# BurntSushi/suffix

Hardware: NVIDIA H100
Metric: MB/s input text indexed (SA+LCP build) (higher is better)
Workload: dtype u32

## Files before the change

suffix_b200/csrc/b200sa.cu:

```cuda
#include <cuda_runtime.h>
#include <stdint.h>
#include <stdio.h>
#include <stdlib.h>
#include <string.h>

#include <string>
#include <vector>

#include "../../include/b200sa.h"
#include "../../include/b200sa_internal.h"
#include "common.cuh"
#include "classify.cuh"
#include "classify2.cuh"
#include "induce.cuh"
#include "induce2.cuh"
#include "induce3.cuh"
#include "induce4.cuh"
#include "induce5.cuh"
#include "induce6.cuh"
#include "pipeline_kernels.cuh"
#include "lms_sort.cuh"
#include "shard.cuh"
#include "tree.cuh"
#include "nccl_dyn.h"
// ... 93 lines not shown

static inline uint32_t cdiv(uint64_t a, uint64_t b) { return (uint32_t)((a + b - 1) / b); }

static int mark(b200sa_ctx *c, const char *name) {
    if (!c->timing) return B200SA_OK;
    if (c->events_used == c->event_pool.size()) {
        cudaEvent_t e;
        CU_TRY(c, cudaEventCreate(&e));
        c->event_pool.push_back(e);
    }
    cudaEvent_t e = c->event_pool[c->events_used++];
    CU_TRY(c, cudaEventRecord(e, c->stream));
    c->marks.push_back({name, e});
    return B200SA_OK;
}
static void begin_call(b200sa_ctx *c, void *stream) {
    c->stream = stream ? (cudaStream_t)stream : c->own_stream;
    c->marks.clear();
    c->events_used = 0;
    c->launches = 0;
    c->last_error.clear();
}
static void l2_window(b200sa_ctx *c, const void *p, size_t bytes);
static int end_call(b200sa_ctx *c) {
    if (c->l2_persist) l2_window(c, nullptr, 0);
    c->stats.kernel_launches = c->launches;
    c->stats.workspace_bytes = c->ws_bytes;
    c->phase_names.clear();
    c->phase_ms.clear();
    if (c->timing && c->marks.size() >= 2) {
        CU_TRY(c, cudaEventSynchronize(c->marks.back().second));
        for (size_t i = 0; i + 1 < c->marks.size(); i++) {
            float ms = 0;
            CU_TRY(c, cudaEventElapsedTime(&ms, c->marks[i].second, c->marks[i + 1].second));
            c->phase_names.push_back(c->marks[i].first);
            c->phase_ms.push_back(ms);
        }
    }
    return B200SA_OK;
}

template <class... KArgs, class... Args>
static inline void launch_k(b200sa_ctx *c, void (*kern)(KArgs...), uint32_t grid, Args... args) {
    kern<<<grid, BLK, 0, c->stream>>>(args...);
    c->launches++;
}
#define LAUNCH(ctx, kern, grid, ...) launch_k((ctx), kern, (grid), __VA_ARGS__)

static int read_words(b200sa_ctx *c, const uint32_t *dsrc, int count) {
    CU_TRY(c, cudaMemcpyAsync(c->h_pin, dsrc, sizeof(uint32_t) * count, cudaMemcpyDeviceToHost, c->stream));
    CU_TRY(c, cudaStreamSynchronize(c->stream));
    return B200SA_OK;
}

static int scan_state_for(b200sa_ctx *c, uint32_t nb, ScanState *S) {
    size_t need = (size_t)nb * 28 + 64;
    if (c->scan_state.cap < need) {
        TRY(ensure(c, c->scan_state, need * 2));
        CU_TRY(c, cudaMemsetAsync(c->scan_state.p, 0, c->scan_state.cap, c->stream));
        c->scan_tiles_cap = (uint32_t)((c->scan_state.cap - 64) / 28);
    }
    uint8_t *basep = ptr<uint8_t>(c->scan_state);
    S->ticket = reinterpret_cast<uint32_t *>(basep);
    S->agg = reinterpret_cast<unsigned long long *>(basep + 64);
    S->incl = S->agg + c->scan_tiles_cap;
    S->pk = S->incl + c->scan_tiles_cap;
    S->flag = reinterpret_cast<uint32_t *>(S->pk + c->scan_tiles_cap);
    c->scan_epoch += 2;
    S->epoch = c->scan_epoch;
    return B200SA_OK;
}

template <class Op, class InF, class OutF>
static int dev_scan(b200sa_ctx *c, InF in, OutF out, uint64_t n, typename Op::T *d_total) {
    typedef typename Op::T T;
    if (n == 0) {
        if (d_total) CU_TRY(c, cudaMemsetAsync(d_total, 0, sizeof(T), c->stream));
        return B200SA_OK;
    }
    uint32_t nb = cdiv(n, SCAN_CHUNK);
    ScanState S;
    TRY(scan_state_for(c, nb, &S));
    LAUNCH(c, (k_scan_lb<Op, InF, OutF>), nb, in, out, n, nb, S, d_total);
    CU_TRY(c, cudaGetLastError());
    return B200SA_OK;
}

static inline uint32_t grid_cap(const b200sa_ctx *c) { return (uint32_t)c->sm_count * 8u; }

template <class DigF, class MoveF>
static int radix_pass(b200sa_ctx *c, DigF dig, MoveF mv, uint64_t n) {
    if (n == 0) return B200SA_OK;
    uint32_t tiles = cdiv(n, TILE);
    uint32_t nb = tiles < grid_cap(c) ? tiles : grid_cap(c);
    uint32_t tpb = cdiv(tiles, nb);
    nb = cdiv(tiles, tpb);
    TRY(ensure(c, c->radix_cnt, (size_t)256 * nb * 4));
    uint32_t *cnt = ptr<uint32_t>(c->radix_cnt);
    LAUNCH(c, (k_radix_hist<DigF>), nb, dig, n, tpb, cnt);
    TRY((dev_scan<OpSum>(c, InArray{cnt}, OutStoreExcl{cnt}, (uint64_t)256 * nb, nullptr)));
    LAUNCH(c, (k_radix_scatter<DigF, MoveF>), nb, dig, mv, n, tpb, cnt);
    CU_TRY(c, cudaGetLastError());
    return B200SA_OK;
}

template <class K, int OSI>
static int sort_pairs_t(b200sa_ctx *c, K *ka, uint32_t *va, K *kb, uint32_t *vb, uint64_t n, int bits,
                      K **kout, uint32_t **vout) {
    *kout = ka;
    *vout = va;
    if (n == 0 || bits <= 0) return B200SA_OK;
    int npass = (bits + 7) / 8;
    if (npass > OS_MAX_PASSES) npass = OS_MAX_PASSES;
    uint32_t tiles = cdiv(n, OSI * BLK);
    size_t status_bytes = (size_t)tiles * 256 * 8;
    TRY(ensure(c, c->os_hist, OS_MAX_PASSES * 256 * 4 + 64));
    TRY(ensure(c, c->os_status, status_bytes));
    uint32_t *ghist = ptr<uint32_t>(c->os_hist);
    uint32_t *ticket = ghist + OS_MAX_PASSES * 256;
    CU_TRY(c, cudaMemsetAsync(ghist, 0, OS_MAX_PASSES * 256 * 4 + 64, c->stream));
    uint32_t hb = cdiv(n, TILE) < grid_cap(c) ? cdiv(n, TILE) : grid_cap(c);
    {
        size_t shm = (size_t)NWARP * npass * 256 * 4;
        auto kfn = k_os_hist<K, LoadArr<K>>;
        CU_TRY(c, cudaFuncSetAttribute(kfn, cudaFuncAttributeMaxDynamicSharedMemorySize, (int)(NWARP * OS_MAX_PASSES * 256 * 4)));
        kfn<<<hb, BLK, shm, c->stream>>>(LoadArr<K>{ka}, n, npass, 0u, ghist, (K *)nullptr);
        c->launches++;
    }
    LAUNCH(c, k_os_scan, (uint32_t)npass, ghist);
    for (int p = 0; p < npass; p++) {
        CU_TRY(c, cudaMemsetAsync(c->os_status.p, 0, status_bytes, c->stream));
        LAUNCH(c, (k_os_pass<K, LoadArr<K>, LoadArr<uint32_t>, OSI>), tiles, LoadArr<K>{ka}, LoadArr<uint32_t>{va}, kb, vb, n,
               (uint32_t)(8 * p), ghist + p * 256,
               reinterpret_cast<volatile unsigned long long *>(c->os_status.p), ticket + p);
        K *tk = ka; ka = kb; kb = tk;
        uint32_t *tv = va; va = vb; vb = tv;
    }
    CU_TRY(c, cudaGetLastError());
    *kout = ka;
    *vout = va;
    return B200SA_OK;
}

template <class K>
static int sort_pairs(b200sa_ctx *c, K *ka, uint32_t *va, K *kb, uint32_t *vb, uint64_t n, int bits,
                      K **kout, uint32_t **vout) {
    if (n >= (1u << 20) && !getenv("B200SA_SORT_NARROW"))
        return sort_pairs_t<K, (sizeof(K) == 4 ? 16 : 12)>(c, ka, va, kb, vb, n, bits, kout, vout);
    return sort_pairs_t<K, ITEMS>(c, ka, va, kb, vb, n, bits, kout, vout);
}

template <class K, class KeyF, class ValF, int OSI = ITEMS>
static int sort_pairs_from(b200sa_ctx *c, KeyF keyf, ValF valf, K *ka, uint32_t *va, K *kb, uint32_t *vb, uint64_t n,
                           int bits, K **kout, uint32_t **vout) {
    *kout = ka;
    *vout = va;
    if (n == 0) return B200SA_OK;
    int npass = (bits + 7) / 8;
    if (npass < 1) npass = 1;
    if (npass > OS_MAX_PASSES) npass = OS_MAX_PASSES;
    uint32_t tiles = cdiv(n, OSI * BLK);
    size_t status_bytes = (size_t)tiles * 256 * 8;
    TRY(ensure(c, c->os_hist, OS_MAX_PASSES * 256 * 4 + 64));
    TRY(ensure(c, c->os_status, status_bytes));
    uint32_t *ghist = ptr<uint32_t>(c->os_hist);
    uint32_t *ticket = ghist + OS_MAX_PASSES * 256;
    CU_TRY(c, cudaMemsetAsync(ghist, 0, OS_MAX_PASSES * 256 * 4 + 64, c->stream));
    uint32_t hb = cdiv(n, TILE) < grid_cap(c) ? cdiv(n, TILE) : grid_cap(c);
    {
        size_t shm = (size_t)NWARP * npass * 256 * 4;
        auto kfn = k_os_hist<K, KeyF>;
        CU_TRY(c, cudaFuncSetAttribute(kfn, cudaFuncAttributeMaxDynamicSharedMemorySize, (int)(NWARP * OS_MAX_PASSES * 256 * 4)));
        kfn<<<hb, BLK, shm, c->stream>>>(keyf, n, npass, 0u, ghist, kb);
        c->launches++;
    }
    LAUNCH(c, k_os_scan, (uint32_t)npass, ghist);
    volatile unsigned long long *status = reinterpret_cast<volatile unsigned long long *>(c->os_status.p);
    CU_TRY(c, cudaMemsetAsync(c->os_status.p, 0, status_bytes, c->stream));
    LAUNCH(c, (k_os_pass<K, LoadArr<K>, ValF, OSI>), tiles, LoadArr<K>{kb}, valf, ka, va, n, 0u, ghist, status, ticket);
    for (int p = 1; p < npass; p++) {
        CU_TRY(c, cudaMemsetAsync(c->os_status.p, 0, status_bytes, c->stream));
        LAUNCH(c, (k_os_pass<K, LoadArr<K>, LoadArr<uint32_t>, OSI>), tiles, LoadArr<K>{ka}, LoadArr<uint32_t>{va}, kb, vb, n,
               (uint32_t)(8 * p), ghist + p * 256, status, ticket + p);
        K *tk = ka; ka = kb; kb = tk;
        uint32_t *tv = va; va = vb; vb = tv;
    }
    CU_TRY(c, cudaGetLastError());
    *kout = ka;
    *vout = va;
    return B200SA_OK;
}

static int bit_length(uint64_t x) {
    int b = 0;
    while (x) { b++; x >>= 1; }
    return b;
}

static int doubling_rounds(b200sa_ctx *c, uint32_t m, uint32_t na, uint32_t *asuf, uint32_t *ascratch, uint64_t h,
                           uint32_t *rounds_io, const uint32_t *names_arr = nullptr, uint32_t kgram = 0,
                           uint32_t bw = 0) {
    uint32_t *sa_r = ptr<uint32_t>(c->sa_r), *rank = ptr<uint32_t>(c->rank);
    uint32_t *apos = ptr<uint32_t>(c->p0), *apos_next = ptr<uint32_t>(c->p1);
    uint32_t *G0 = ptr<uint32_t>(c->g0), *G1 = ptr<uint32_t>(c->g1), *agrp = G0;
    uint32_t *d_na = ptr<uint32_t>(c->small);
    uint32_t rounds = *rounds_io;
    if (na > 0) {
        TRY(ensure(c, c->k64a, (size_t)na * 8));
        TRY(ensure(c, c->k64b, (size_t)na * 8));
    }
    int b2 = bit_length(m);
    bool try_local = getenv("B200SA_NO_LOCAL_SORT") == nullptr;
    static const char *kSortNames[] = {"rsa_sort1", "rsa_sort2", "rsa_sort3", "rsa_sort4", "rsa_sort5", "rsa_sortN"};
    static const char *kScanNames[] = {"rsa_scan1", "rsa_scan2", "rsa_scan3", "rsa_scan4", "rsa_scan5", "rsa_scanN"};
    while (na > 0) {
        rounds++;
        { uint32_t ri = rounds - *rounds_io; TRY(mark(c, kSortNames[ri <= 5 ? ri - 1 : 5])); }
        if (rounds > 40) { c->last_error = "doubling did not converge"; return B200SA_ERR_INTERNAL; }
        uint64_t *KA = ptr<uint64_t>(c->k64a), *KB = ptr<uint64_t>(c->k64b), *K2;
        uint32_t hh = h > 0xffffffffull ? 0xffffffffu : (uint32_t)h;
        bool first = (names_arr != nullptr) && rounds == *rounds_io + 1 && kgram >= 2;
        int bits = 2 * b2;
        if (first) {
            LAUNCH(c, (k_multi_key_list<uint64_t>), cdiv(na, BLK), names_arr, m, asuf, na, kgram, bw, KA);
            bits = (int)(kgram * bw);
        } else {
            LAUNCH(c, k_pair_keys, cdiv(na, BLK), agrp, asuf, rank, na, m, hh, (uint32_t)b2, KA);
        }
        uint32_t *Vsorted = nullptr;
        bool sorted_locally = false;
        bool use_local = !first && try_local;
        if (use_local) {
            CU_TRY(c, cudaMemsetAsync(d_na + 24, 0, 16, c->stream));
            uint32_t stride = na / 4096u; if (stride < 1) stride = 1;
            uint32_t samples = cdiv(na, stride);
            LAUNCH(c, k_group_probe, cdiv(samples, BLK), KA, na, (uint32_t)b2, stride, d_na + 25);
            TRY(read_words(c, d_na + 25, 2));
            if (c->h_pin[0] * 20u > samples) use_local = false;
        }
        if (use_local) {
            LAUNCH(c, k_group_local_sort, cdiv(na, BLK), KA, asuf, na, (uint32_t)b2, KB, ascratch, d_na + 24);
            TRY(read_words(c, d_na + 24, 1));
            if (c->h_pin[0] == 0) { K2 = KB; Vsorted = ascratch; sorted_locally = true; }
            else try_local = false;
        }
        if (!sorted_locally) TRY(sort_pairs<uint64_t>(c, KA, asuf, KB, ascratch, na, bits, &K2, &Vsorted));
        uint32_t *Vother = (Vsorted == asuf) ? ascratch : asuf;
        { uint32_t ri = rounds - *rounds_io; TRY(mark(c, kScanNames[ri <= 5 ? ri - 1 : 5])); }
        TRY((dev_scan<OpMaxSum>(c, InGroupActive<uint64_t>{K2, apos, na},
                                OutGroupRankCompact{Vsorted, apos, rank, sa_r, apos_next, Vother, G0}, na,
                                reinterpret_cast<unsigned long long *>(d_na + 16))));
        TRY(read_words(c, d_na + 16, 1));
        na = c->h_pin[0];
        if (getenv("B200SA_TRACE")) fprintf(stderr, "[b200sa] doubling round %u: h=%llu -> active %u of %u\n", rounds, (unsigned long long)h, na, m);
        asuf = Vother; ascratch = Vsorted;
        uint32_t *t = apos; apos = apos_next; apos_next = t;
        agrp = G0;
        if (first) h = kgram; else h *= 2;
    }
    *rounds_io = rounds;
    return B200SA_OK;
}


static int reduced_sa(b200sa_ctx *c, uint32_t *R, uint32_t m, uint32_t names, uint32_t *rounds_out) {
    TRY(ensure(c, c->sa_r, (size_t)m * 4));
    TRY(ensure(c, c->k32b, (size_t)m * 4));
    TRY(ensure(c, c->v0, (size_t)m * 4));
    TRY(ensure(c, c->v1, (size_t)m * 4));
    TRY(ensure(c, c->p0, (size_t)m * 4));
    TRY(ensure(c, c->p1, (size_t)m * 4));
    TRY(ensure(c, c->g0, (size_t)m * 4));
    TRY(ensure(c, c->g1, (size_t)m * 4));
    TRY(ensure(c, c->rank, (size_t)m * 4));
    TRY(ensure(c, c->small, 256));
    uint32_t *sa_r = ptr<uint32_t>(c->sa_r), *rank = ptr<uint32_t>(c->rank);
    uint32_t *V0 = ptr<uint32_t>(c->v0), *V1 = ptr<uint32_t>(c->v1);
    uint32_t *P0 = ptr<uint32_t>(c->p0), *P1 = ptr<uint32_t>(c->p1);
    uint32_t *G0 = ptr<uint32_t>(c->g0), *G1 = ptr<uint32_t>(c->g1);
    uint32_t *d_na = ptr<uint32_t>(c->small);
    uint32_t rounds = 0;

    LAUNCH(c, k_iota, cdiv(m, BLK), V0, m);
    int bm = bit_length(m);
    int bw = bit_length(names);
    if (bw < 1) bw = 1;
    uint32_t k0 = 1;
    if (bw + 3 < bm) {
        k0 = (uint32_t)((bm + 2 + bw - 1) / bw);
        if ((int)k0 * bw > 64) k0 = 64 / bw;
    }
    if (const char *e = getenv("B200SA_K0")) { int v = atoi(e); if (v >= 1 && v * bw <= 64) k0 = (uint32_t)v; }
    uint32_t *Vs;
    uint32_t na = 0;
    if ((int)k0 * bw <= 32) {
        uint32_t *KA = ptr<uint32_t>(c->k32b), *Ks;
        LAUNCH(c, (k_multi_key<uint32_t>), cdiv(m, BLK), R, m, k0, (uint32_t)bw, KA);
        TRY(sort_pairs<uint32_t>(c, KA, V0, R, V1, m, (int)k0 * bw, &Ks, &Vs));
        TRY((dev_scan<OpMax>(c, InGroupStart<uint32_t>{Ks, nullptr}, OutGroupRank{Vs, nullptr, G1, rank, sa_r}, m, nullptr)));
        uint32_t *Vf = (Vs == V0) ? V1 : V0;
        TRY((dev_scan<OpSum>(c, InActive<uint32_t>{Ks, m}, OutCompactActive{nullptr, Vs, G1, P0, Vf, G0}, m, d_na)));
    } else {
        TRY(ensure(c, c->k64a, (size_t)m * 8));
        TRY(ensure(c, c->k64b, (size_t)m * 8));
        uint64_t *KA = ptr<uint64_t>(c->k64a), *KB = ptr<uint64_t>(c->k64b), *Ks;
        LAUNCH(c, (k_multi_key<uint64_t>), cdiv(m, BLK), R, m, k0, (uint32_t)bw, KA);
        TRY(sort_pairs<uint64_t>(c, KA, V0, KB, V1, m, (int)k0 * bw, &Ks, &Vs));
        TRY((dev_scan<OpMax>(c, InGroupStart<uint64_t>{Ks, nullptr}, OutGroupRank{Vs, nullptr, G1, rank, sa_r}, m, nullptr)));
        uint32_t *Vf = (Vs == V0) ? V1 : V0;
        TRY((dev_scan<OpSum>(c, InActive<uint64_t>{Ks, m}, OutCompactActive{nullptr, Vs, G1, P0, Vf, G0}, m, d_na)));
    }
    uint32_t *Vfree = (Vs == V0) ? V1 : V0;
    TRY(read_words(c, d_na, 1));
    na = c->h_pin[0];
    TRY(doubling_rounds(c, m, na, Vfree, Vs, k0, &rounds));
    if (rounds_out) *rounds_out = rounds;
    return B200SA_OK;
}

static void l2_window(b200sa_ctx *c, const void *p, size_t bytes) {
    if (!c->l2_persist || c->l2_max_window == 0) return;
    cudaStreamAttrValue v;
    memset(&v, 0, sizeof v);
    v.accessPolicyWindow.base_ptr = const_cast<void *>(p);
    v.accessPolicyWindow.num_bytes = bytes < c->l2_max_window ? bytes : c->l2_max_window;
    v.accessPolicyWindow.hitRatio = bytes ? 1.0f : 0.0f;
    v.accessPolicyWindow.hitProp = cudaAccessPropertyPersisting;
    v.accessPolicyWindow.missProp = cudaAccessPropertyStreaming;
    if (cudaStreamSetAttribute(c->stream, cudaStreamAttributeAccessPolicyWindow, &v) != cudaSuccess) cudaGetLastError();
}

static int pack_text(b200sa_ctx *c, const uint8_t *text, uint64_t n, uint32_t sigma) {
    uint32_t *tab = ptr<uint32_t>(c->tables);
    c->bits = 8;
    c->ptext = text;
    c->sigma = sigma;
    if (getenv("B200SA_NOPACK")) return B200SA_OK;
    if (sigma <= 4) c->bits = 2; else if (sigma <= 16) c->bits = 4; else return B200SA_OK;
    uint32_t cpw = 32 / c->bits;
    uint64_t words = (n + cpw - 1) / cpw;
    TRY(ensure(c, c->packed, words * 4 + 32));
    if (c->bits == 2) LAUNCH(c, (k_pack<2>), cdiv(words, BLK), text, n, tab + T_CODE, ptr<uint32_t>(c->packed));
    else LAUNCH(c, (k_pack<4>), cdiv(words, BLK), text, n, tab + T_CODE, ptr<uint32_t>(c->packed));
    CU_TRY(c, cudaGetLastError());
    c->ptext = c->packed.p;
    if (words * 4 <= c->l2_set_aside) l2_window(c, c->packed.p, words * 4 + 8);
    return B200SA_OK;
}

static uint32_t window_chars(uint32_t sigma, int bits, uint64_t *range_out) {
    if (bits == 2) { *range_out = 1ull << 32; return 16; }
    if (sigma < 2) sigma = 2;
    uint32_t cap = bits == 4 ? 13u : 8u, k = 0;
    uint64_t r = 1;
    while (k < cap && r * sigma <= (1ull << 32)) { r *= sigma; k++; }
    *range_out = r;
    return k;
}

template <int BITS>
static int lms_direct_sort_t(b200sa_ctx *c, uint32_t n, uint32_t m, uint32_t **list_out, bool *done) {
    *done = false;
    uint64_t range = 0;
    LmsWin W;
    W.ptext = c->ptext; W.code_of = ptr<uint32_t>(c->tables) + T_CODE; W.n = n;
    W.sigma = BITS == 2 ? 4u : c->sigma;
    W.kc = window_chars(c->sigma, BITS, &range);
    const uint32_t kc = W.kc;
    TRY(ensure(c, c->k32b, (size_t)m * 4));
    TRY(ensure(c, c->reduced, (size_t)m * 4));
    TRY(ensure(c, c->v0, (size_t)m * 4));
    TRY(ensure(c, c->v1, (size_t)m * 4));
    TRY(ensure(c, c->small, 4096));
    uint32_t *sm = ptr<uint32_t>(c->small);
    uint32_t *Ks, *Ps;
    TRY(mark(c, "lms_sort"));
    {
        const char *e = getenv("B200SA_SORT_ITEMS");
        const bool wide = e ? atoi(e) == 16 : (m >= (1u << 20) && !getenv("B200SA_SORT_NARROW"));
        LmsKeyDesc<BITS> kf{W, ptr<uint32_t>(c->lmsdesc)};
        LmsValDesc vf{ptr<uint32_t>(c->lmsdesc)};
        if (wide)
            TRY((sort_pairs_from<uint32_t, LmsKeyDesc<BITS>, LmsValDesc, 16>(c, kf, vf, ptr<uint32_t>(c->k32b), ptr<uint32_t>(c->v0),
                                                                             ptr<uint32_t>(c->reduced), ptr<uint32_t>(c->v1), m,
                                                                             bit_length(range - 1), &Ks, &Ps)));
        else
            TRY((sort_pairs_from<uint32_t, LmsKeyDesc<BITS>, LmsValDesc, ITEMS>(c, kf, vf, ptr<uint32_t>(c->k32b), ptr<uint32_t>(c->v0),
                                                                                ptr<uint32_t>(c->reduced), ptr<uint32_t>(c->v1), m,
                                                                                bit_length(range - 1), &Ks, &Ps)));
    }
    TRY(mark(c, "lms_groups"));
    TRY(ensure(c, c->p0, (size_t)m * 4));
    TRY(ensure(c, c->p1, (size_t)m * 4));
    TRY(ensure(c, c->g0, (size_t)m * 4));
    TRY(ensure(c, c->g1, (size_t)m * 4));
    TRY(ensure(c, c->sa_r, (size_t)m * 4));
    TRY(ensure(c, c->rank, (size_t)m * 4));
    uint32_t *slotA = ptr<uint32_t>(c->p0), *slotB = ptr<uint32_t>(c->p1);
    uint32_t *grpA = ptr<uint32_t>(c->g0), *grpB = ptr<uint32_t>(c->g1);
    uint32_t *posA = ptr<uint32_t>(c->sa_r), *posB = ptr<uint32_t>(c->rank);
    unsigned long long *d_tot = reinterpret_cast<unsigned long long *>(sm + 16);
    {
        size_t fw = ((size_t)m + 31) / 32 + 1;
        TRY(ensure(c, c->flag, fw * 4));
        uint32_t *forced = ptr<uint32_t>(c->flag);
        CU_TRY(c, cudaMemsetAsync(forced, 0, fw * 4, c->stream));
        CU_TRY(c, cudaMemsetAsync(sm + 16, 0, 8, c->stream));
        LAUNCH(c, (k_lms_mark_trunc<BITS>), 1u, W, ptr<uint32_t>(c->lmsdesc), m, Ks, Ps, kc, forced);
        if (getenv("B200SA_GROUPS_GENERIC")) {
            InLmsActive1 in1{Ks, forced, m};
            TRY((dev_scan<OpSum>(c, in1, OutLmsCompact1{in1, Ps, slotA, posA, grpA}, m, sm + 16)));
        } else {
            uint32_t nt = cdiv(m, LG_TILE);
            ScanState S;
            TRY(scan_state_for(c, nt, &S));
            LAUNCH(c, k_lms_groups1, nt, Ks, Ps, forced, m, nt, S, slotA, posA, grpA, sm + 16);
            CU_TRY(c, cudaGetLastError());
        }
    }
    TRY(read_words(c, sm + 16, 1));
    uint32_t na = c->h_pin[0];
    c->stats.names = m - na;
    uint32_t rounds = 1;
    uint32_t max_rounds = BITS == 8 ? 16u : 8u;
    if (const char *e = getenv("B200SA_DIRECT_ROUNDS")) { int v = atoi(e); if (v >= 1) max_rounds = (uint32_t)v; }
    if (getenv("B200SA_TRACE")) fprintf(stderr, "[b200sa] direct LMS sort: kc=%u, round 1 leaves %u of %u tied\n", kc, na, m);
    const bool force = getenv("B200SA_DIRECT_FORCE") != nullptr;
    if (!force && (uint64_t)na * 1000 > (uint64_t)m * 999 && m > 64) return B200SA_OK;
    if (na > 0)
        TRY((dev_scan<OpMax>(c, InArray{grpA}, OutMaxInPlace{grpA}, na, nullptr)));
    uint64_t h = kc;
    const bool allow_local = getenv("B200SA_NO_LOCAL_SORT") == nullptr;
    const int gbits = 32 + bit_length(m);
    while (na > 0) {
        if (rounds >= max_rounds) return B200SA_OK;
        rounds++;
        {
            static const char *kNames[] = {"lms_refine2", "lms_refine3", "lms_refine4", "lms_refine5", "lms_refineN"};
            TRY(mark(c, kNames[rounds - 2 < 4 ? rounds - 2 : 4]));
        }
        TRY(ensure(c, c->k64a, (size_t)na * 8));
        TRY(ensure(c, c->k64b, (size_t)na * 8));
        TRY(ensure(c, c->sorted, (size_t)m * 4));
        uint64_t *KA = ptr<uint64_t>(c->k64a), *KB = ptr<uint64_t>(c->k64b), *K2 = nullptr;
        uint32_t *scratch = ptr<uint32_t>(c->sorted), *P2 = nullptr;
        LAUNCH(c, (k_lms_refine_keys<BITS>), cdiv(na, BLK), W, posA, grpA, na, (uint32_t)h, KA);
        const uint32_t span = (uint32_t)(h + kc > 0xffffffffull ? 0xffffffffull : h + kc);
        bool local_ok = false;
        bool try_local = allow_local;
        if (try_local && na >= (1u << 20)) {
            CU_TRY(c, cudaMemsetAsync(sm + 24, 0, 16, c->stream));
            uint32_t stride = na / 4096u; if (stride < 1) stride = 1;
            uint32_t samples = cdiv(na, stride);
            LAUNCH(c, k_group_probe, cdiv(samples, BLK), KA, na, 32u, stride, sm + 25);
            TRY(read_words(c, sm + 25, 2));
            if (c->h_pin[0] * 20u > samples) try_local = false;
        }
        if (try_local) {
            CU_TRY(c, cudaMemsetAsync(sm + 24, 0, 4, c->stream));
            LAUNCH(c, k_group_local_sort, cdiv(na, BLK), KA, posA, na, 32u, KB, scratch, sm + 24);
            TRY((dev_scan<OpMaxSum>(c, InLmsGroupR{KB, scratch, slotA, na, n, span},
                                    OutLmsCompactR{scratch, slotA, Ps, slotB, posB, grpB}, na, d_tot)));
            TRY(read_words(c, sm + 16, 9));
            local_ok = c->h_pin[8] == 0;
        }
        if (!local_ok) {
            TRY(sort_pairs<uint64_t>(c, KA, posA, KB, scratch, na, gbits, &K2, &P2));
            TRY((dev_scan<OpMaxSum>(c, InLmsGroupR{K2, P2, slotA, na, n, span},
                                    OutLmsCompactR{P2, slotA, Ps, slotB, posB, grpB}, na, d_tot)));
            TRY(read_words(c, sm + 16, 1));
        }
        uint32_t na_next = c->h_pin[0];
        if (getenv("B200SA_TRACE")) fprintf(stderr, "[b200sa] direct LMS sort: round %u (h=%llu): %u -> %u tied\n", rounds, (unsigned long long)h, na, na_next);
        if (!force && (uint64_t)na_next * 100 > (uint64_t)na * 85 && (uint64_t)na_next * 64 > m) return B200SA_OK;
        na = na_next;
        uint32_t *t;
        t = slotA; slotA = slotB; slotB = t;
        t = posA; posA = posB; posB = t;
        t = grpA; grpA = grpB; grpB = t;
        h += kc;
    }
    c->stats.doubling_rounds = rounds;
    *list_out = Ps;
    *done = true;
    return B200SA_OK;
}
static int lms_direct_sort(b200sa_ctx *c, uint32_t n, uint32_t m, uint32_t **list_out, bool *done) {
    if (c->bits == 2) return lms_direct_sort_t<2>(c, n, m, list_out, done);
    if (c->bits == 4) return lms_direct_sort_t<4>(c, n, m, list_out, done);
    return lms_direct_sort_t<8>(c, n, m, list_out, done);
}

static int induce_variant_env() {
    const char *e = getenv("B200SA_INDUCE");
    return e ? atoi(e) : 0;
}
static int induce_variant(int bits) {
    int v = induce_variant_env();
    if (v == 2 && bits < 8) return 2;
    if (v == 1) return 1;
    if (bits == 2) return (v >= 3 && v <= 5) ? v : 6;
    return 1;
}
static const void *induce_fn_v(bool spass, int bits, int variant) {
    if (variant == 6 && bits == 2) return spass ? (const void *)k_induce6<true> : (const void *)k_induce6<false>;
    if (variant == 5 && bits == 2) return spass ? (const void *)k_induce5<true> : (const void *)k_induce5<false>;
    if (variant == 4 && bits == 2) return spass ? (const void *)k_induce4<true> : (const void *)k_induce4<false>;
    if (variant == 3 && bits == 2) return spass ? (const void *)k_induce3<true> : (const void *)k_induce3<false>;
    if (variant == 2 && bits == 2) return spass ? (const void *)k_induce2<true, 2> : (const void *)k_induce2<false, 2>;
    if (variant == 2 && bits == 4) return spass ? (const void *)k_induce2<true, 4> : (const void *)k_induce2<false, 4>;
    if (bits == 2) return spass ? (const void *)k_induce<true, 2> : (const void *)k_induce<false, 2>;
    if (bits == 4) return spass ? (const void *)k_induce<true, 4> : (const void *)k_induce<false, 4>;
    return spass ? (const void *)k_induce<true, 8> : (const void *)k_induce<false, 8>;
}
static int launch_induce(b200sa_ctx *c, bool spass, const uint8_t *text, uint32_t n, uint32_t *sa,
                         const uint32_t *lms, uint32_t m) {
    (void)m;
    uint32_t *tab = ptr<uint32_t>(c->tables);
    InduceArgs A;
    A.text = text; A.ptext = c->ptext; A.alpha = tab + T_ALPHA;
    A.n = n; A.sa = sa; A.pred = ptr<uint8_t>(c->pred);
    A.lms = lms; A.lms_pred = ptr<uint8_t>(c->lmspred);
    A.bstart = tab + T_BSTART; A.Lcnt = tab + T_LCNT; A.Scnt = tab + T_SCNT; A.lms_off = tab + T_LMSOFF;
    A.blk_cnt = ptr<uint32_t>(c->blkcnt);
    uint32_t *sm = ptr<uint32_t>(c->small);
    A.g_fill = sm + 64; A.g_state = reinterpret_cast<int32_t *>(sm + 320); A.err = sm + 32;
    A.run_scratch = ptr<uint32_t>(c->runscr);
    A.run_alive = A.run_scratch + TILE;
    A.cmd = sm + 336;
    A.steplog = nullptr;
    A.blocklog_step = 0;
    A.carry = 0;
    { static int rs = -1; if (rs < 0) { const char *e = getenv("B200SA_RUN_STREAK"); rs = e ? atoi(e) : 0; } A.run_streak = (uint32_t)rs; }
    if (getenv("B200SA_STEPLOG")) {
        if (ensure(c, c->steplog, 8192 * 8) == B200SA_OK) {
            A.steplog = ptr<unsigned long long>(c->steplog);
            if (const char *e = getenv("B200SA_BLOCKLOG")) {
                int ps = 0, st = 0;
                if (sscanf(e, "%d:%d", &ps, &st) == 2 && ps == (spass ? 1 : 0)) A.blocklog_step = (uint32_t)st + 1u;
            }
            if (!spass) cudaMemsetAsync(c->steplog.p, 0, 8, c->stream);
        }
    }
    void *args[] = {&A};
    int variant = induce_variant(c->bits);
    if (variant >= 3 && (((uintptr_t)sa | (uintptr_t)lms) & 15) != 0) variant = 1;
    A.carry = (variant >= 5) ? 2 : (variant == 4 ? 1 : 0);
    int bi = c->bits == 2 ? 0 : (c->bits == 4 ? 1 : 2);
    int blocks = c->cur_induce_blocks, cap = c->sm_count * c->induce_occ_v[variant][bi];
    if (blocks > cap) blocks = cap;
    A.cascade = 0;
    if (variant == 6 && !getenv("B200SA_NO_CASCADE")) {
        A.cascade = (uint32_t)blocks * (uint32_t)TILE;
        if (const char *e = getenv("B200SA_CASCADE_MAX")) { long v = atol(e); if (v >= 0 && (uint64_t)v < A.cascade) A.cascade = (uint32_t)v; }
    }
    CU_TRY(c, cudaLaunchCooperativeKernel(induce_fn_v(spass, c->bits, variant), dim3(blocks), dim3(BLK), args, 0, c->stream));
    c->launches++;
    return B200SA_OK;
}

static int post_classify(b200sa_ctx *c, const uint8_t *text, uint64_t n, uint32_t sigma) {
    TRY(pack_text(c, text, n, sigma));
    int bps = sigma <= 16 ? 3 : (sigma <= 64 ? 2 : 1);
    if (c->induce_bps_env) bps = c->induce_bps_env;
    int occ_here = c->induce_occ[c->bits == 2 ? 0 : (c->bits == 4 ? 1 : 2)];
    if (bps > occ_here) bps = occ_here;
    if (bps < 1) bps = 1;
    c->cur_induce_blocks = c->sm_count * bps;
    return B200SA_OK;
}

static int classify_fused_dev(b200sa_ctx *c, const uint8_t *text, uint64_t n, uint32_t *m_out,
                              ShardEdge edge = ShardEdge{-1, -1, ST_L}, bool pack = true) {
    uint64_t nw = (n + 31) / 32;
    uint32_t nbc = cdiv(nw, CLS_WORDS);
    TRY(ensure(c, c->stype, nw * 4));
    TRY(ensure(c, c->lmsb, nw * 4));
    TRY(ensure(c, c->tables, T_END * 4));
    TRY(ensure(c, c->small, 4096));
    TRY(ensure(c, c->lmsdesc, (size_t)(n / 2 + 2) * 4));
    if (c->cls_state.cap < (size_t)nbc * 4) {
        TRY(ensure(c, c->cls_state, (size_t)nbc * 8));
// ... 1300 lines not shown
```

suffix_b200/csrc/lms_sort.cuh:

```cuda
#pragma once
#include "classify.cuh"

namespace b200sa {

struct LmsWin {
    const void *ptext;
    const uint32_t *code_of;
    uint32_t n, sigma, kc;
};

__device__ __forceinline__ uint32_t rev_pairs(uint32_t x) {
    uint32_t y = __brev(x);
    return ((y & 0x55555555u) << 1) | ((y >> 1) & 0x55555555u);
}

template <int BITS>
__device__ __forceinline__ uint32_t lms_window(const LmsWin &W, uint32_t p) {
    const uint32_t left = W.n - p;
    if (BITS == 2) {
        if (left == 0) return 0u;
        uint32_t x = text_bits<2>(W.ptext, p);
        if (left < 16u) x &= (1u << (2u * left)) - 1u;
        return rev_pairs(x);
    } else if (BITS == 4) {
        if (left == 0) return 0u;
        uint32_t lo = text_bits<4>(W.ptext, p);
        uint32_t hi = (W.kc > 8u && left > 8u) ? text_bits<4>(W.ptext, p + 8u) : 0u;
        uint32_t key = 0;
        for (uint32_t i = 0; i < W.kc; i++) {
            uint32_t c = (i < 8u ? (lo >> (4u * i)) : (hi >> (4u * (i - 8u)))) & 15u;
            key = key * W.sigma + (i < left ? c : 0u);
        }
        return key;
    } else {
        const uint8_t *t = reinterpret_cast<const uint8_t *>(W.ptext);
        uint32_t key = 0;
        if (W.sigma == 256u) {
#pragma unroll
            for (uint32_t i = 0; i < 4u; i++) key = (key << 8) | (i < left ? (uint32_t)__ldg(t + p + i) : 0u);
            return key;
        }
        for (uint32_t i = 0; i < W.kc; i++) {
            uint32_t c = i < left ? __ldg(W.code_of + __ldg(t + p + i)) : 0u;
            key = key * W.sigma + c;
        }
        return key;
    }
}

template <int BITS>
struct LmsKeyDesc {
    LmsWin W; const uint32_t *lmsdesc;
    __device__ __forceinline__ uint32_t operator()(uint64_t i) const { return lms_window<BITS>(W, __ldg(lmsdesc + i)); }
    __device__ __forceinline__ uint32_t at(uint64_t, uint32_t pos) const { return lms_window<BITS>(W, pos); }
};
struct LmsValDesc {
    const uint32_t *lmsdesc;
    __device__ __forceinline__ uint32_t operator()(uint64_t i) const { return __ldg(lmsdesc + i); }
};

template <int BITS>
__global__ void __launch_bounds__(BLK) k_lms_mark_trunc(LmsWin W, const uint32_t *__restrict__ lmsdesc, uint32_t m,
                                                        const uint32_t *__restrict__ K, const uint32_t *__restrict__ P,
                                                        uint32_t span, uint32_t *forced) {
    uint32_t t = threadIdx.x;
    if (t >= m || t >= span) return;
    uint32_t p = lmsdesc[t];
    if ((uint64_t)p + span <= W.n) return;
    uint32_t key = lms_window<BITS>(W, p);
    uint32_t lo = 0, hi = m;
    while (lo < hi) {
        uint32_t mid = lo + (hi - lo) / 2;
        if (K[mid] < key) lo = mid + 1; else hi = mid;
    }
    for (uint32_t j = lo; j < m && K[j] == key; j++) {
        if (P[j] == p) {
            atomicOr(&forced[j >> 5], 1u << (j & 31));
            if (j + 1 < m) atomicOr(&forced[(j + 1) >> 5], 1u << ((j + 1) & 31));
            break;
        }
    }
}
struct InLmsActive1 {
    const uint32_t *K, *forced; uint32_t m;
    __device__ __forceinline__ bool head(uint32_t i) const {
        uint32_t a = K[i], b = K[i > 0 ? i - 1 : 0], f = forced[i >> 5];
        return (i == 0) | (a != b) | ((f >> (i & 31)) & 1u);
    }
    __device__ __forceinline__ uint32_t operator()(uint64_t ii) const {
        uint32_t i = (uint32_t)ii, j = i + 1 < m ? i + 1 : i;
        uint32_t a = K[i], b = K[i > 0 ? i - 1 : 0], c = K[j], f = forced[i >> 5], f2 = forced[j >> 5];
        bool hd = (i == 0) | (a != b) | ((f >> (i & 31)) & 1u);
        bool tl = (i + 1 == m) | (c != a) | ((f2 >> (j & 31)) & 1u);
        return (hd & tl) ? 0u : 1u;
    }
};
struct OutLmsCompact1 {
    InLmsActive1 in; const uint32_t *P; uint32_t *aslot, *apos, *ahead;
    __device__ void operator()(uint64_t i, uint32_t exc, uint32_t v) const {
        if (v) { aslot[exc] = (uint32_t)i; apos[exc] = P[i]; ahead[exc] = in.head((uint32_t)i) ? (uint32_t)i : 0u; }
    }
};
constexpr int LG_IPT = 16;
constexpr int LG_TILE = BLK * LG_IPT;
__global__ void __launch_bounds__(BLK) k_lms_groups1(const uint32_t *__restrict__ K, const uint32_t *__restrict__ P,
                                                     const uint32_t *__restrict__ forced, uint32_t m, uint32_t ntiles,
                                                     ScanState S, uint32_t *aslot, uint32_t *apos, uint32_t *ahead,
                                                     uint32_t *d_total) {
    __shared__ uint32_t s_w[NWARP + 1];
    __shared__ uint32_t s_tile, s_prefix;
    if (threadIdx.x == 0) {
        uint32_t t = atomicAdd(S.ticket, 1u);
        if (t + 1 == ntiles) *S.ticket = 0u;
        s_tile = t;
    }
    __syncthreads();
    const uint32_t tile = s_tile;
    const uint32_t i0 = tile * LG_TILE + threadIdx.x * LG_IPT;
    uint32_t k[LG_IPT + 2];
    if (i0 + LG_IPT <= m) {
        const uint4 *q = reinterpret_cast<const uint4 *>(K + i0);
#pragma unroll
        for (int v = 0; v < 4; v++) {
            uint4 a = __ldg(q + v);
            k[1 + 4 * v] = a.x; k[2 + 4 * v] = a.y; k[3 + 4 * v] = a.z; k[4 + 4 * v] = a.w;
        }
    } else {
#pragma unroll
        for (int j = 0; j < LG_IPT; j++) k[1 + j] = (i0 + j < m) ? __ldg(K + i0 + j) : 0u;
    }
    k[0] = (i0 > 0 && i0 <= m) ? __ldg(K + i0 - 1) : 0u;
    k[LG_IPT + 1] = (i0 + LG_IPT < m) ? __ldg(K + i0 + LG_IPT) : 0u;
    uint32_t fw = (i0 < m) ? __ldg(forced + (i0 >> 5)) : 0u;
    uint32_t fbits = (fw >> (i0 & 31)) & 0xffffu;
    if (i0 + LG_IPT < m) {
        uint32_t nxt = ((i0 & 31) == 16) ? __ldg(forced + (i0 >> 5) + 1) : (fw >> 16);
        fbits |= (nxt & 1u) << 16;
    }
    uint32_t head = 0;
#pragma unroll
    for (int j = 0; j <= LG_IPT; j++) {
        uint32_t i = i0 + j;
        bool h = (i == 0) | (i >= m) | (k[j + 1] != k[j]) | ((fbits >> j) & 1u);
        head |= (h ? 1u : 0u) << j;
    }
    uint32_t act = 0;
#pragma unroll
    for (int j = 0; j < LG_IPT; j++) {
        bool a = (i0 + j < m) && !(((head >> j) & 1u) && ((head >> (j + 1)) & 1u));
        act |= (a ? 1u : 0u) << j;
    }
    uint32_t cnt = __popc(act), btot;
    uint32_t inc = block_incl_scan<OpSum>(cnt, s_w, &btot);
    if (warp_id() == 0) {
        if (lane_id() == 0) tile_publish_u32(S, tile, btot);
        uint32_t prefix = tile_walk_u32(S, tile, btot, tile + 1 == ntiles, d_total);
        if (lane_id() == 0) s_prefix = prefix;
    }
    __syncthreads();
    uint32_t at = s_prefix + inc - cnt;
    while (act) {
        uint32_t j = __ffs(act) - 1;
        act &= act - 1;
        uint32_t i = i0 + j;
        aslot[at] = i; apos[at] = __ldg(P + i); ahead[at] = ((head >> j) & 1u) ? i : 0u;
        at++;
    }
}

struct OutMaxInPlace {
    uint32_t *a;
    __device__ void operator()(uint64_t i, uint32_t exc, uint32_t v) const { a[i] = exc > v ? exc : v; }
};

template <int BITS>
__global__ void __launch_bounds__(BLK) k_lms_refine_keys(LmsWin W, const uint32_t *__restrict__ apos,
                                                         const uint32_t *__restrict__ agrp, uint32_t na, uint32_t h,
                                                         uint64_t *keys) {
    uint32_t j = blockIdx.x * BLK + threadIdx.x;
    if (j >= na) return;
    keys[j] = ((uint64_t)agrp[j] << 32) | lms_window<BITS>(W, apos[j] + h);
}
struct InLmsGroupR {
    const uint64_t *K; const uint32_t *P, *slot; uint32_t na, n, span;
    __device__ __forceinline__ bool trunc(uint32_t p) const { return (uint64_t)p + span > n; }
    __device__ __forceinline__ bool head(uint32_t j) const {
        return j == 0 || K[j] != K[j - 1] || trunc(P[j - 1]) || trunc(P[j]);
    }
    __device__ unsigned long long operator()(uint64_t jj) const {
        uint32_t j = (uint32_t)jj;
        bool hd = head(j), tl = (j + 1 == na) || head(j + 1);
        return ((unsigned long long)(hd ? slot[j] : 0u) << 32) | ((hd && tl) ? 0u : 1u);
    }
};
struct OutLmsCompactR {
    const uint32_t *P, *slot; uint32_t *list; uint32_t *oslot, *opos, *ogrp;
    __device__ void operator()(uint64_t j, unsigned long long exc, unsigned long long v) const {
        uint32_t p = P[j], sl = slot[j];
        list[sl] = p;
        if ((uint32_t)v) {
            uint32_t eh = (uint32_t)(exc >> 32), vh = (uint32_t)(v >> 32), k = (uint32_t)exc;
            oslot[k] = sl; opos[k] = p; ogrp[k] = eh > vh ? eh : vh;
        }
    }
};

}
```

Baseline: 16080.

## Replace four-pass LMS radix sort with top-16 pass plus in-tile bucket sort

For the 2-bit alphabet, the LMS window sort now radix-sorts only the top 16 key bits in global memory. A new per-tile kernel then finishes each top-16 bucket in shared memory, using either a counting sort or a local multi-pass radix sort. The same kernel fuses group-head detection, tied-suffix compaction and the decoupled-lookback scan, which removes the separate groups kernel and the max scan. If any bucket exceeds the shared-memory capacity, it falls back to the original full four-pass sort. That fallback risks redoing the work.

```diff
diff --git a/suffix_b200/csrc/b200sa.cu b/suffix_b200/csrc/b200sa.cu
--- a/suffix_b200/csrc/b200sa.cu
+++ b/suffix_b200/csrc/b200sa.cu
@@ -269,7 +269,7 @@
 
 template <class K, class KeyF, class ValF, int OSI = ITEMS>
 static int sort_pairs_from(b200sa_ctx *c, KeyF keyf, ValF valf, K *ka, uint32_t *va, K *kb, uint32_t *vb, uint64_t n,
-                           int bits, K **kout, uint32_t **vout) {
+                           int bits, K **kout, uint32_t **vout, uint32_t shift0 = 0) {
     *kout = ka;
     *vout = va;
     if (n == 0) return B200SA_OK;
@@ -288,17 +288,17 @@
         size_t shm = (size_t)NWARP * npass * 256 * 4;
         auto kfn = k_os_hist<K, KeyF>;
         CU_TRY(c, cudaFuncSetAttribute(kfn, cudaFuncAttributeMaxDynamicSharedMemorySize, (int)(NWARP * OS_MAX_PASSES * 256 * 4)));
-        kfn<<<hb, BLK, shm, c->stream>>>(keyf, n, npass, 0u, ghist, kb);
+        kfn<<<hb, BLK, shm, c->stream>>>(keyf, n, npass, shift0, ghist, kb);
         c->launches++;
     }
     LAUNCH(c, k_os_scan, (uint32_t)npass, ghist);
     volatile unsigned long long *status = reinterpret_cast<volatile unsigned long long *>(c->os_status.p);
     CU_TRY(c, cudaMemsetAsync(c->os_status.p, 0, status_bytes, c->stream));
-    LAUNCH(c, (k_os_pass<K, LoadArr<K>, ValF, OSI>), tiles, LoadArr<K>{kb}, valf, ka, va, n, 0u, ghist, status, ticket);
+    LAUNCH(c, (k_os_pass<K, LoadArr<K>, ValF, OSI>), tiles, LoadArr<K>{kb}, valf, ka, va, n, shift0, ghist, status, ticket);
     for (int p = 1; p < npass; p++) {
         CU_TRY(c, cudaMemsetAsync(c->os_status.p, 0, status_bytes, c->stream));
         LAUNCH(c, (k_os_pass<K, LoadArr<K>, LoadArr<uint32_t>, OSI>), tiles, LoadArr<K>{ka}, LoadArr<uint32_t>{va}, kb, vb, n,
-               (uint32_t)(8 * p), ghist + p * 256, status, ticket + p);
+               shift0 + (uint32_t)(8 * p), ghist + p * 256, status, ticket + p);
         K *tk = ka; ka = kb; kb = tk;
         uint32_t *tv = va; va = vb; vb = tv;
     }
@@ -491,22 +491,6 @@
     TRY(ensure(c, c->small, 4096));
     uint32_t *sm = ptr<uint32_t>(c->small);
     uint32_t *Ks, *Ps;
-    TRY(mark(c, "lms_sort"));
-    {
-        const char *e = getenv("B200SA_SORT_ITEMS");
-        const bool wide = e ? atoi(e) == 16 : (m >= (1u << 20) && !getenv("B200SA_SORT_NARROW"));
-        LmsKeyDesc<BITS> kf{W, ptr<uint32_t>(c->lmsdesc)};
-        LmsValDesc vf{ptr<uint32_t>(c->lmsdesc)};
-        if (wide)
-            TRY((sort_pairs_from<uint32_t, LmsKeyDesc<BITS>, LmsValDesc, 16>(c, kf, vf, ptr<uint32_t>(c->k32b), ptr<uint32_t>(c->v0),
-                                                                             ptr<uint32_t>(c->reduced), ptr<uint32_t>(c->v1), m,
-                                                                             bit_length(range - 1), &Ks, &Ps)));
-        else
-            TRY((sort_pairs_from<uint32_t, LmsKeyDesc<BITS>, LmsValDesc, ITEMS>(c, kf, vf, ptr<uint32_t>(c->k32b), ptr<uint32_t>(c->v0),
-                                                                                ptr<uint32_t>(c->reduced), ptr<uint32_t>(c->v1), m,
-                                                                                bit_length(range - 1), &Ks, &Ps)));
-    }
-    TRY(mark(c, "lms_groups"));
     TRY(ensure(c, c->p0, (size_t)m * 4));
     TRY(ensure(c, c->p1, (size_t)m * 4));
     TRY(ensure(c, c->g0, (size_t)m * 4));
@@ -517,7 +501,54 @@
     uint32_t *grpA = ptr<uint32_t>(c->g0), *grpB = ptr<uint32_t>(c->g1);
     uint32_t *posA = ptr<uint32_t>(c->sa_r), *posB = ptr<uint32_t>(c->rank);
     unsigned long long *d_tot = reinterpret_cast<unsigned long long *>(sm + 16);
-    {
+    const char *items_env = getenv("B200SA_SORT_ITEMS");
+    const bool wide = items_env ? atoi(items_env) == 16 : (m >= (1u << 20) && !getenv("B200SA_SORT_NARROW"));
+    LmsKeyDesc<BITS> kf{W, ptr<uint32_t>(c->lmsdesc)};
+    LmsValDesc vf{ptr<uint32_t>(c->lmsdesc)};
+    bool bucketed = false;
+    if (BITS == 2 && !getenv("B200SA_LMS_SORT4")) {
+        TRY(mark(c, "lms_sort"));
+        if (wide)
+            TRY((sort_pairs_from<uint32_t, LmsKeyDesc<BITS>, LmsValDesc, 16>(c, kf, vf, ptr<uint32_t>(c->k32b), ptr<uint32_t>(c->v0),
+                                                                             ptr<uint32_t>(c->reduced), ptr<uint32_t>(c->v1), m,
+                                                                             16, &Ks, &Ps, 16u)));
+        else
+            TRY((sort_pairs_from<uint32_t, LmsKeyDesc<BITS>, LmsValDesc, ITEMS>(c, kf, vf, ptr<uint32_t>(c->k32b), ptr<uint32_t>(c->v0),
+                                                                                ptr<uint32_t>(c->reduced), ptr<uint32_t>(c->v1), m,
+                                                                                16, &Ks, &Ps, 16u)));
+        TRY(mark(c, "lms_groups"));
+        uint32_t *Pout = ptr<uint32_t>(c->k32b);
+        CU_TRY(c, cudaMemsetAsync(sm + 16, 0, 12, c->stream));
+        uint32_t nt = cdiv(m, BS_T);
+        ScanState S;
+        TRY(scan_state_for(c, nt, &S));
+        CU_TRY(c, cudaFuncSetAttribute(k_lms_bucket_sort, cudaFuncAttributeMaxDynamicSharedMemorySize, (int)BS_SMEM));
+        CU_TRY(c, cudaFuncSetAttribute(k_lms_bucket_sort, cudaFuncAttributePreferredSharedMemoryCarveout, 100));
+        if (getenv("B200SA_TRACE")) {
+            int occ = 0;
+            cudaOccupancyMaxActiveBlocksPerMultiprocessor(&occ, k_lms_bucket_sort, BLK, BS_SMEM);
+            fprintf(stderr, "[b200sa] k_lms_bucket_sort: %u CTAs, %d per SM\n", nt, occ);
+        }
+        k_lms_bucket_sort<<<nt, BLK, BS_SMEM, c->stream>>>(Ks, Ps, m, n, kc, nt, S, Pout, slotA, posA, grpA, sm + 16, sm + 18);
+        c->launches++;
+        CU_TRY(c, cudaGetLastError());
+        TRY(read_words(c, sm + 16, 3));
+        bucketed = c->h_pin[2] == 0;
+        Ps = Pout;
+        if (!bucketed && getenv("B200SA_TRACE"))
+            fprintf(stderr, "[b200sa] direct LMS sort: a top-16 bucket holds more than %u suffixes: four-pass sort\n", BS_CAP);
+    }
+    if (!bucketed) {
+        TRY(mark(c, "lms_sort"));
+        if (wide)
+            TRY((sort_pairs_from<uint32_t, LmsKeyDesc<BITS>, LmsValDesc, 16>(c, kf, vf, ptr<uint32_t>(c->k32b), ptr<uint32_t>(c->v0),
+                                                                             ptr<uint32_t>(c->reduced), ptr<uint32_t>(c->v1), m,
+                                                                             bit_length(range - 1), &Ks, &Ps)));
+        else
+            TRY((sort_pairs_from<uint32_t, LmsKeyDesc<BITS>, LmsValDesc, ITEMS>(c, kf, vf, ptr<uint32_t>(c->k32b), ptr<uint32_t>(c->v0),
+                                                                                ptr<uint32_t>(c->reduced), ptr<uint32_t>(c->v1), m,
+                                                                                bit_length(range - 1), &Ks, &Ps)));
+        TRY(mark(c, "lms_groups"));
         size_t fw = ((size_t)m + 31) / 32 + 1;
         TRY(ensure(c, c->flag, fw * 4));
         uint32_t *forced = ptr<uint32_t>(c->flag);
@@ -534,17 +565,18 @@
             LAUNCH(c, k_lms_groups1, nt, Ks, Ps, forced, m, nt, S, slotA, posA, grpA, sm + 16);
             CU_TRY(c, cudaGetLastError());
         }
-    }
-    TRY(read_words(c, sm + 16, 1));
+        TRY(read_words(c, sm + 16, 1));
+    }
     uint32_t na = c->h_pin[0];
     c->stats.names = m - na;
     uint32_t rounds = 1;
     uint32_t max_rounds = BITS == 8 ? 16u : 8u;
     if (const char *e = getenv("B200SA_DIRECT_ROUNDS")) { int v = atoi(e); if (v >= 1) max_rounds = (uint32_t)v; }
-    if (getenv("B200SA_TRACE")) fprintf(stderr, "[b200sa] direct LMS sort: kc=%u, round 1 leaves %u of %u tied\n", kc, na, m);
+    if (getenv("B200SA_TRACE")) fprintf(stderr, "[b200sa] direct LMS sort: kc=%u, round 1 leaves %u of %u tied%s\n", kc, na, m,
+                                        bucketed ? " (bucket sort)" : "");
     const bool force = getenv("B200SA_DIRECT_FORCE") != nullptr;
     if (!force && (uint64_t)na * 1000 > (uint64_t)m * 999 && m > 64) return B200SA_OK;
-    if (na > 0)
+    if (na > 0 && !bucketed)
         TRY((dev_scan<OpMax>(c, InArray{grpA}, OutMaxInPlace{grpA}, na, nullptr)));
     uint64_t h = kc;
     const bool allow_local = getenv("B200SA_NO_LOCAL_SORT") == nullptr;
diff --git a/suffix_b200/csrc/lms_sort.cuh b/suffix_b200/csrc/lms_sort.cuh
--- a/suffix_b200/csrc/lms_sort.cuh
+++ b/suffix_b200/csrc/lms_sort.cuh
@@ -168,6 +168,283 @@
     }
 }
 
+constexpr uint32_t BS_T = 4096;
+constexpr uint32_t BS_CAP = 4096;
+constexpr uint32_t BS_SPAN_MAX = BS_T + BS_CAP;
+constexpr uint32_t BS_ROUNDS = BS_SPAN_MAX / BLK;
+constexpr size_t BS_SMEM = (size_t)BS_SPAN_MAX * (4 + 2 + 2);
+constexpr uint32_t BS_BIN_MAX = 64;
+__global__ void __launch_bounds__(BLK, 3) k_lms_bucket_sort(const uint32_t *__restrict__ K, const uint32_t *__restrict__ P,
+                                                            uint32_t m, uint32_t n, uint32_t kc, uint32_t ntiles,
+                                                            ScanState S, uint32_t *Pout, uint32_t *aslot,
+                                                            uint32_t *apos, uint32_t *ahead, uint32_t *d_total,
+                                                            uint32_t *d_over) {
+    extern __shared__ uint32_t s_dyn[];
+    uint32_t *s_key = s_dyn;
+    uint16_t *s_ia = reinterpret_cast<uint16_t *>(s_dyn + BS_SPAN_MAX);
+    uint16_t *s_ib = s_ia + BS_SPAN_MAX;
+    __shared__ __align__(16) uint32_t s_wcnt[NWARP][256];
+    __shared__ uint32_t s_base[256], s_hist[256];
+    unsigned long long *s_seg = reinterpret_cast<unsigned long long *>(&s_wcnt[0][0]);
+    __shared__ unsigned long long s_w64[NWARP + 1];
+    __shared__ uint32_t s_w[NWARP + 1];
+    __shared__ uint32_t s_tile, s_lo, s_hi, s_over, s_prefix;
+    const uint32_t tid = threadIdx.x, w = warp_id(), l = lane_id();
+    if (tid == 0) {
+        uint32_t t = atomicAdd(S.ticket, 1u);
+        if (t + 1 == ntiles) *S.ticket = 0u;
+        s_tile = t; s_lo = m; s_hi = m; s_over = 0u;
+    }
+    __syncthreads();
+    const uint32_t tile = s_tile;
+    const uint32_t w0 = tile * BS_T, w1 = min(w0 + BS_T, m);
+    const uint32_t e = min(m, w0 + BS_SPAN_MAX);
+    const uint32_t kprev = w0 > 0 ? __ldg(K + w0 - 1) >> 16 : 0xffffffffu;
+    if (e - w0 == BS_SPAN_MAX) {
+        const uint4 *q = reinterpret_cast<const uint4 *>(K + w0);
+        uint4 v[BS_SPAN_MAX / 4 / BLK];
+#pragma unroll
+        for (int k = 0; k < (int)(BS_SPAN_MAX / 4 / BLK); k++) v[k] = __ldg(q + k * BLK + tid);
+#pragma unroll
+        for (int k = 0; k < (int)(BS_SPAN_MAX / 4 / BLK); k++) reinterpret_cast<uint4 *>(s_key)[k * BLK + tid] = v[k];
+    } else {
+        for (uint32_t i = tid; i < e - w0; i += BLK) s_key[i] = __ldg(K + w0 + i);
+    }
+    __syncthreads();
+    for (uint32_t i = tid; i < w1 - w0; i += BLK) {
+        uint32_t hi16 = s_key[i] >> 16, pr = i > 0 ? s_key[i - 1] >> 16 : kprev;
+        if (pr != hi16) {
+            atomicMin(&s_lo, w0 + i);
+            if (w0 + i + BS_CAP < m && (s_key[i + BS_CAP] >> 16) == hi16) atomicOr(&s_over, 1u);
+        }
+    }
+    __syncthreads();
+    const bool work = s_lo < w1 && s_over == 0u;
+    if (s_over && tid == 0) *d_over = 1u;
+    if (work) {
+        for (uint32_t i = w1 - w0 + tid; i < e - w0; i += BLK)
+            if ((s_key[i] >> 16) != (s_key[i - 1] >> 16)) atomicMin(&s_hi, w0 + i);
+        __syncthreads();
+    }
+    const uint32_t lo = s_lo, len = work ? s_hi - lo : 0u;
+    const uint32_t R = (len + BLK - 1) / BLK;
+    uint32_t *sk = s_key + (lo - w0);
+    uint32_t hb = 0;
+    uint32_t tb = 0;
+    unsigned long long seg_total = 0;
+    uint16_t *src = s_ia;
+    if (work) {
+        uint32_t pv[BS_ROUNDS];
+#pragma unroll
+        for (uint32_t r = 0; r < BS_ROUNDS; r++) {
+            if (r >= R) break;
+            uint32_t j = r * BLK + tid;
+            pv[r] = j < len ? __ldg(P + lo + j) : 0u;
+        }
+        for (uint32_t r = 0; r < R; r++) {
+            uint32_t j = r * BLK + tid;
+            bool h = j < len && (j == 0 || (sk[j] >> 16) != (sk[j - 1] >> 16));
+            hb |= (h ? 1u : 0u) << r;
+            uint32_t bal = __ballot_sync(FULL, h);
+            if (l == 0) s_hist[r * NWARP + w] = __popc(bal);
+        }
+        __syncthreads();
+        uint32_t nb;
+        {
+            uint32_t v = tid < R * NWARP ? s_hist[tid] : 0u;
+            uint32_t inc = block_incl_scan<OpSum>(v, s_w, &nb);
+            s_hist[tid] = inc - v;
+        }
+        __syncthreads();
+#pragma unroll
+        for (uint32_t r = 0; r < BS_ROUNDS; r++) {
+            if (r >= R) break;
+            uint32_t j = r * BLK + tid;
+            uint32_t bal = __ballot_sync(FULL, (hb >> r) & 1u);
+            uint32_t ord = s_hist[r * NWARP + w] + __popc(bal & (lanemask_lt() | (1u << l))) - 1u;
+            if (j < len) sk[j] = (ord << 16) | (sk[j] & 0xffffu) | (((uint64_t)pv[r] + kc > n) ? 0x80000000u : 0u);
+        }
+        __syncthreads();
+        const int ob = nb > 1 ? 32 - __clz(nb - 1) : 0;
+        bool sorted = false;
+        if (ob <= 10) {
+            uint32_t *s_bin = &s_wcnt[0][0];
+            const int lb = 11 - ob;
+            for (uint32_t i = tid; i < 2048u; i += BLK) s_bin[i] = 0;
+            __syncthreads();
+#pragma unroll 4
+            for (uint32_t j = tid; j < len; j += BLK) {
+                uint32_t k = sk[j] & 0x7fffffffu;
+                atomicAdd(&s_bin[((k >> 16) << lb) | ((k & 0xffffu) >> (16 - lb))], 1u);
+            }
+            __syncthreads();
+            uint32_t c[8], sum = 0, mx = 0;
+#pragma unroll
+            for (int q = 0; q < 8; q++) { c[q] = s_bin[tid * 8 + q]; sum += c[q]; mx = max(mx, c[q]); }
+            uint32_t tot;
+            uint32_t run = block_incl_scan<OpSum>(sum, s_w, &tot) - sum;
+#pragma unroll
+            for (int q = 0; q < 8; q++) { s_bin[tid * 8 + q] = run; run += c[q]; }
+            if (!__syncthreads_or(mx > BS_BIN_MAX)) {
+                uint32_t *s_pk = reinterpret_cast<uint32_t *>(s_ia);
+                const uint32_t lmask = (1u << (16 - lb)) - 1u;
+#pragma unroll 4
+                for (uint32_t j = tid; j < len; j += BLK) {
+                    uint32_t k = sk[j] & 0x7fffffffu;
+                    s_pk[atomicAdd(&s_bin[((k >> 16) << lb) | ((k & 0xffffu) >> (16 - lb))], 1u)] = ((k & lmask) << 13) | j;
+                }
+                __syncthreads();
+                uint32_t fin[BS_ROUNDS];
+#pragma unroll
+                for (uint32_t r = 0; r < BS_ROUNDS; r++) {
+                    if (r >= R) break;
+                    uint32_t j = r * BLK + tid;
+                    fin[r] = 0xffffffffu;
+                    if (j < len) {
+                        uint32_t x = s_pk[j], k = sk[x & 0x1fffu] & 0x7fffffffu;
+                        uint32_t b = ((k >> 16) << lb) | ((k & 0xffffu) >> (16 - lb));
+                        uint32_t bs = b ? s_bin[b - 1] : 0u, be = s_bin[b], rank = 0;
+                        for (uint32_t q = bs; q < be; q++) rank += s_pk[q] < x ? 1u : 0u;
+                        fin[r] = ((bs + rank) << 16) | (x & 0x1fffu);
+                    }
+                }
+                __syncthreads();
+#pragma unroll
+                for (uint32_t r = 0; r < BS_ROUNDS; r++) {
+                    if (r >= R) break;
+                    if (fin[r] != 0xffffffffu) s_ia[fin[r] >> 16] = (uint16_t)(fin[r] & 0xffffu);
+                }
+                __syncthreads();
+                sorted = true;
+            }
+        }
+        const int kbits = 16 + (nb > 1 ? 32 - __clz(nb - 1) : 0);
+        const int npass = sorted ? 0 : (kbits + 7) / 8;
+        const uint32_t C = (len + NWARP * 32 - 1) / (NWARP * 32) * 32, RW = C / 32;
+        const uint32_t lt = lanemask_lt();
+        uint16_t *dst = s_ib;
+        for (int p = 0; p < npass; p++) {
+            const uint32_t sh = 8u * p;
+            const int dbits = min(8, kbits - 8 * p);
+#pragma unroll
+            for (int ww = 0; ww < NWARP; ww++) s_wcnt[ww][tid] = 0;
+            __syncthreads();
+            uint32_t pk[BS_ROUNDS];
+#pragma unroll
+            for (uint32_t r = 0; r < BS_ROUNDS; r++) {
+                if (r >= RW) break;
+                uint32_t j = w * C + r * 32 + l;
+                bool v = j < len;
+                uint32_t it = v ? (p == 0 ? j : src[j]) : 0u;
+                uint32_t d = v ? ((sk[it] & 0x7fffffffu) >> sh) & 0xffu : 0u;
+                uint32_t peers = __ballot_sync(FULL, v);
+#pragma unroll
+                for (int b = 0; b < 8; b++) {
+                    if (b >= dbits) break;
+                    uint32_t bal = __ballot_sync(FULL, (d >> b) & 1u);
+                    peers &= ((d >> b) & 1u) ? bal : ~bal;
+                }
+                uint32_t below = __popc(peers & lt);
+                uint32_t base = v ? s_wcnt[w][d] : 0u;
+                __syncwarp();
+                if (v && below == 0) s_wcnt[w][d] = base + __popc(peers);
+                __syncwarp();
+                pk[r] = it | (d << 13) | ((base + below) << 21);
+            }
+            __syncthreads();
+            {
+                uint32_t run = 0;
+#pragma unroll
+                for (int ww = 0; ww < NWARP; ww++) {
+                    uint32_t t = s_wcnt[ww][tid];
+                    s_wcnt[ww][tid] = run;
+                    run += t;
+                }
+                uint32_t tot;
+                uint32_t inc = block_incl_scan<OpSum>(run, s_w, &tot);
+                s_base[tid] = inc - run;
+            }
+            __syncthreads();
+#pragma unroll
+            for (uint32_t r = 0; r < BS_ROUNDS; r++) {
+                if (r >= RW) break;
+                if (w * C + r * 32 + l < len) {
+                    uint32_t d = (pk[r] >> 13) & 0xffu;
+                    dst[s_base[d] + s_wcnt[w][d] + (pk[r] >> 21)] = (uint16_t)(pk[r] & 0x1fffu);
+                }
+            }
+            __syncthreads();
+            uint16_t *t = src; src = dst; dst = t;
+        }
+        for (uint32_t r = 0; r < R; r++) {
+            uint32_t j = r * BLK + tid;
+            bool h = false, tl = true;
+            uint32_t kj = j < len ? sk[src[j]] : 0u;
+            uint32_t kp = __shfl_up_sync(FULL, kj, 1), kn = __shfl_down_sync(FULL, kj, 1);
+            if (j < len) {
+                if (l == 0 && j > 0) kp = sk[src[j - 1]];
+                if (l == 31 && j + 1 < len) kn = sk[src[j + 1]];
+                h = j == 0 || kj != kp || ((kj | kp) >> 31);
+                tl = j + 1 == len || kj != kn || ((kj | kn) >> 31);
+            }
+            bool tied = j < len && !(h && tl);
+            uint32_t balh = __ballot_sync(FULL, h), balt = __ballot_sync(FULL, tied);
+            hb = (hb & ~(1u << r)) | ((h ? 1u : 0u) << r);
+            tb |= (tied ? 1u : 0u) << r;
+            if (l == 0) {
+                uint32_t last = balh ? r * BLK + w * 32 + 31 - __clz(balh) : 0u;
+                s_seg[r * NWARP + w] = ((unsigned long long)last << 32) | __popc(balt);
+            }
+        }
+        __syncthreads();
+        {
+            unsigned long long v = tid < R * NWARP ? s_seg[tid] : 0ull;
+            unsigned long long inc = block_incl_scan<OpMaxSum>(v, s_w64, &seg_total);
+            unsigned long long prev = __shfl_up_sync(FULL, inc, 1);
+            unsigned long long exc = l == 0 ? s_w64[w] : prev;
+            __syncthreads();
+            s_seg[tid] = exc;
+        }
+    }
+    if (tid == 0) tile_publish_u32(S, tile, (uint32_t)seg_total);
+    if (work) {
+        uint32_t pv[BS_ROUNDS];
+#pragma unroll
+        for (uint32_t r = 0; r < BS_ROUNDS; r++) {
+            if (r >= R) break;
+            uint32_t j = r * BLK + tid;
+            pv[r] = j < len ? __ldg(P + lo + j) : 0u;
+        }
+#pragma unroll
+        for (uint32_t r = 0; r < BS_ROUNDS; r++) {
+            if (r >= R) break;
+            uint32_t j = r * BLK + tid;
+            if (j < len) sk[j] = pv[r];
+        }
+        __syncthreads();
+        for (uint32_t j = tid; j < len; j += BLK) Pout[lo + j] = sk[src[j]];
+    }
+    if (w == 0) {
+        uint32_t prefix = tile_walk_u32(S, tile, (uint32_t)seg_total, tile + 1 == ntiles, d_total);
+        if (l == 0) s_prefix = prefix;
+    }
+    __syncthreads();
+    if (!__any_sync(FULL, tb != 0u)) return;
+    const uint32_t prefix = s_prefix;
+    for (uint32_t r = 0; r < R; r++) {
+        uint32_t balh = __ballot_sync(FULL, (hb >> r) & 1u), balt = __ballot_sync(FULL, (tb >> r) & 1u);
+        if (!((tb >> r) & 1u)) continue;
+        const uint32_t j = r * BLK + tid;
+        unsigned long long e = s_seg[r * NWARP + w];
+        uint32_t le = balh & (lanemask_lt() | (1u << l));
+        uint32_t head = le ? r * BLK + w * 32 + 31 - __clz(le) : (uint32_t)(e >> 32);
+        uint32_t at = prefix + (uint32_t)e + __popc(balt & lanemask_lt());
+        aslot[at] = lo + j;
+        apos[at] = Pout[lo + j];
+        ahead[at] = lo + head;
+    }
+}
+
 struct OutMaxInPlace {
     uint32_t *a;
     __device__ void operator()(uint64_t i, uint32_t exc, uint32_t v) const { a[i] = exc > v ? exc : v; }
```

After: 17280 (median of 6 runs). 1.07x the previous value.
